# nelpy/ghost

Hardware: NVIDIA B200
Metric: cwt_output_coeffs_per_sec (higher is better)
Workload: dtype f32

## Files before the change

### ghost_b200/csrc/fast_path.cu

```cuda
#include "plan.h"
#include "common.cuh"
#include "multiplier.cuh"
#include <algorithm>
#include <atomic>
#include <cmath>
#include <cstdio>
#include <cstdlib>
#include <map>
#include <type_traits>

namespace gcwt {

constexpr int kMaxFastLevel = 14;
constexpr int kMaxFullScales = 64;
constexpr double kMaxHaloFrac = 0.45;

__constant__ float c_halfband[kHalfbandOdd];
constexpr int kSmallCoef = (2 + 4 + 8) * kInterpT;
__constant__ float c_interp_small[kSmallCoef];
constexpr int kWideCoef = (4 + 8) * kWideT;
__constant__ float c_interp_wide[kWideCoef];

static double bessel_i0(double x) {
    double sum = 1.0, term = 1.0;
    const double q = x * x / 4.0;
    for (int k = 1; k < 200; ++k) {
        term *= q / ((double)k * (double)k);
        sum += term;
        if (term < 1e-18 * sum) break;
    }
    return sum;
}

static void design_halfband(double* odd ) {
    const int T = kHalfbandT;
    const double atten = 140.0;
    const double beta = 0.1102 * (atten - 8.7);
    const double i0b = bessel_i0(beta);
    double sum = 0.0;
    for (int k = 0; k < kHalfbandOdd; ++k) {
        const int t = 2 * k + 1;
        const double r = (double)t / (double)T;
        const double win = bessel_i0(beta * std::sqrt(std::max(0.0, 1.0 - r * r))) / i0b;
        const double x = M_PI * t / 2.0;
        odd[k] = 0.5 * std::sin(x) / x * win;
        sum += 2.0 * odd[k];
    }
    for (int k = 0; k < kHalfbandOdd; ++k) odd[k] *= 0.5 / sum;
    long double done = 0.0L;
    for (int k = 0; k < kHalfbandOdd; ++k) {
        long double rest = 0.0L;
        for (int j = k + 1; j < kHalfbandOdd; ++j) rest += (long double)odd[j];
        const float f = (float)(0.25L - done - rest);
        odd[k] = (double)f;
        done += (long double)f;
    }
}

static double halfband_gain(const double* odd, double theta) {
    double g = 0.5;
    for (int k = 0; k < kHalfbandOdd; ++k) g += 2.0 * (double)(float)odd[k] * std::cos((2 * k + 1) * theta);
    return g;
}

constexpr int kPlanLevels = kMaxFastLevel - kMinFastLevel + 1;
constexpr int kWide2Levels = kWideMaxLevel - kMinFastLevel + 1;
constexpr int kPlanRow = kPlanLevels * kBins + kFullN + kWide2Levels * 2 * kBins;
// ... 11 lines not shown
        const int k = i - kPlanLevels * kBins - kFullN;
        n = (int64_t)(2 * kChunkDec) << (kMinFastLevel + k / (2 * kBins)); m = k % (2 * kBins);
    }
    out[(int64_t)s * kPlanRow + i] = morse_response(m, n, sc.L, sc.k_first, sc.n_terms, terms + sc.term_off);
}

struct PlanResponses {
    std::vector<double> g;
    const double* level(int s, int lev) const { return g.data() + (size_t)s * kPlanRow + (size_t)(lev - kMinFastLevel) * kBins; }
    const double* full(int s) const { return g.data() + (size_t)s * kPlanRow + (size_t)kPlanLevels * kBins; }
    const double* wide2(int s, int lev) const {
        return g.data() + (size_t)s * kPlanRow + (size_t)kPlanLevels * kBins + kFullN + (size_t)(lev - kMinFastLevel) * 2 * kBins;
    }
};

static int compute_plan_responses(const gcwt_plan* p, PlanResponses& pr) {
    const size_t count = (size_t)p->n_scales * kPlanRow;
    double* d = nullptr;
    GCWT_CUDA_OK(cudaMalloc((void**)&d, sizeof(double) * count));
    plan_response_kernel<<<dim3((kPlanRow + 127) / 128, p->n_scales), 128>>>(p->d_scales, p->d_terms, d);
    count_launch();
    pr.g.resize(count);
    cudaError_t e = cudaMemcpy(pr.g.data(), d, sizeof(double) * count, cudaMemcpyDeviceToHost);
    cudaFree(d);
    if (e != cudaSuccess) { set_error(std::string("plan responses: ") + cudaGetErrorString(e)); return GCWT_ERR_CUDA; }
    return GCWT_OK;
}

static double filter_energy(const gcwt_plan* p, const ScaleInfo& sc, int64_t n) {
    const double* X = p->terms.data() + sc.term_off;
    double e = 0.0;
    for (int t = 0; t < sc.n_terms; ++t) e += X[t] * X[t];
    return e * (double)n / (double)sc.L;
}

static bool band_fits(const gcwt_plan* p, const PlanResponses& pr, int s, int level) {
    const double* g = pr.level(s, level);
    double e_in = 0.0;
    for (int m = 0; m < kBins; ++m) e_in += g[m] * g[m];
    const double e_tot = filter_energy(p, p->scales[s], (int64_t)kChunkDec << level);
    return (1.0 - e_in / e_tot) < p->band_tol * p->band_tol;
}

static int full_extent(const gcwt_plan* p, const PlanResponses& pr, int s) {
    const double* g = pr.full(s);
    const double e_tot = filter_energy(p, p->scales[s], kFullN);
    double e_in = 0.0;
    int m = 0;
    for (int nmu = 2; nmu <= 8; nmu *= 2) {
        for (; m < nmu * kBins; ++m) e_in += g[m] * g[m];
        if ((1.0 - e_in / e_tot) < p->band_tol * p->band_tol) return nmu;
    }
    return 16;
}

static int band_width_bins(const gcwt_plan* p, const PlanResponses& pr, int s, int level) {
    const double* g = pr.level(s, level);
    const double e_tot = filter_energy(p, p->scales[s], (int64_t)kChunkDec << level);
    const double budget = 0.5 * p->band_tol * p->band_tol * e_tot;
    int lo = 0, hi = kBins - 1;
    double acc = 0.0;
    while (lo < hi && acc + g[lo] * g[lo] < budget) { acc += g[lo] * g[lo]; ++lo; }
    acc = 0.0;
    while (hi > lo && acc + g[hi] * g[hi] < budget) { acc += g[hi] * g[hi]; --hi; }
    return hi - lo + 1;
}

static int choose_level(const gcwt_plan* p, const PlanResponses& pr, int s) {
    const ScaleInfo& sc = p->scales[s];
    if (!(p->flags & GCWT_FLAG_FORCE_GENERIC)) {
        int lo = kMinFastLevel;
        while (lo <= kMaxFastLevel && (double)(sc.L - 1) > kMaxHaloFrac * (double)((int64_t)kChunkDec << lo)) ++lo;
        int hi = std::min(kMaxFastLevel, ilog2_ceil(sc.L) + 1);
        for (int lev = hi; lev >= lo; --lev)
            if (band_fits(p, pr, s, lev)) return lev;
        if ((double)(sc.L - 1) <= kMaxHaloFrac * kFullN) return -1;
    }
    return -2;
}

static void class_geometry(FastClass& fc) {
    const int64_t d = fc.level >= 0 ? (int64_t(1) << fc.level) : 1;
    const int64_t align = std::max<int64_t>(d, 16);
    const int taps = fc.wide ? kWideT : kInterpT;
    const int64_t lead = fc.interp ? (int64_t)(taps / 2 - 1) << fc.log2u : 0;
    const int64_t tail = fc.interp ? (int64_t)(taps / 2 + 1) << fc.log2u : 0;
    fc.offset = ((fc.lmax / 2 + lead + align - 1) / align) * align;
    fc.hop = ((fc.nc_full - (fc.lmax - 1) / 2 - tail - fc.offset) / align) * align;
}

static long double sinc_pi(long double x) {
    const long double pi = 3.14159265358979323846264338327950288L;
    return x == 0.0L ? 1.0L : sinl(pi * x) / (pi * x);
}

static void design_interpolator(int log2u, std::vector<float>& coef, int T, double os) {
    const int U = 1 << log2u;
    const long double fmax = 0.5L / (long double)os;
    coef.resize((size_t)U * T);
    std::vector<long double> A((size_t)T * T), b(T);
    for (int t = 0; t < T; ++t) coef[t] = (t == T / 2 - 1) ? 1.f : 0.f;
    for (int phi = 1; phi < U; ++phi) {
        for (int t = 0; t < T; ++t) {
            const long double dt = (long double)(t - (T / 2 - 1)) - (long double)phi / U;
            for (int u = 0; u < T; ++u) A[(size_t)t * T + u] = sinc_pi(2.0L * fmax * (long double)(t - u));
            b[t] = sinc_pi(2.0L * fmax * dt);
// ... 106 lines not shown
            const double step = 2.0 * pi / (double)sc.L;
            double far = 0.0, near = 0.0;
            for (int q = 0; q < sc.n_terms; ++q) {
                const int64_t k = sc.k_first + q;
                const double d = w - step * (double)k;
                if (fabs(d) < step) near += X[q];
                else far += ((k & 1) ? -X[q] : X[q]) / sin(0.5 * d);
            }
            const double v = 1.15 * (fabs(far) / (double)sc.L + near);
            atomicMax(&mx[b], __float_as_uint((float)v));
        }
    }
    __syncthreads();
    if (tid < kGuardSlots) out[(int64_t)s * kGuardSlots + tid] = __uint_as_float(mx[tid]);
}

static int guard_plan_build(gcwt_plan* p, const PlanResponses& pr, const std::vector<double>& hb) {
    const int S = p->n_scales;
    std::vector<float> gain((size_t)S * kGuardSlots, 0.f), q(S, 0.f);
    std::vector<int32_t> cls(S, -1);
    for (size_t ci = 0; ci < p->classes.size(); ++ci)
        for (int id : p->classes[ci].scale_ids) cls[id] = (int32_t)ci;
    GCWT_CUDA_OK(cudaMemcpy(p->d_scales, p->scales.data(), sizeof(ScaleInfo) * S, cudaMemcpyHostToDevice));
    float* d_drop = nullptr;
    GCWT_CUDA_OK(cudaMalloc((void**)&d_drop, sizeof(float) * S * kGuardSlots));
    guard_drop_kernel<<<S, 256>>>(p->d_scales, p->d_terms, d_drop);
    count_launch();
    std::vector<float> drop((size_t)S * kGuardSlots);
    cudaError_t e = cudaMemcpy(drop.data(), d_drop, sizeof(float) * drop.size(), cudaMemcpyDeviceToHost);
    cudaFree(d_drop);
    if (e != cudaSuccess) { set_error(std::string("guard tables: ") + cudaGetErrorString(e)); return GCWT_ERR_CUDA; }
    HbTaps taps;
    for (int k = 0; k < kHalfbandOdd; ++k) taps.odd[k] = (double)(float)p->halfband_odd[k];
    std::map<int, std::vector<float>> alias;
    for (const FastClass& fc : p->classes) {
        if (fc.level < kMinFastLevel || alias.count(fc.level)) continue;
        unsigned* d_b = nullptr;
        GCWT_CUDA_OK(cudaMalloc((void**)&d_b, sizeof(unsigned) * kGuardSlots * kBins));
        GCWT_CUDA_OK(cudaMemset(d_b, 0, sizeof(unsigned) * kGuardSlots * kBins));
        const int64_t total = (int64_t)kBins << fc.level;
        guard_alias_kernel<<<(unsigned)((total + 255) / 256), 256>>>(fc.level, taps, d_b);
        count_launch();
        std::vector<float>& B = alias[fc.level];
        B.resize((size_t)kGuardSlots * kBins);
        e = cudaMemcpy(B.data(), d_b, sizeof(float) * B.size(), cudaMemcpyDeviceToHost);
        cudaFree(d_b);
        if (e != cudaSuccess) { set_error(std::string("guard tables: ") + cudaGetErrorString(e)); return GCWT_ERR_CUDA; }
    }
    for (int s = 0; s < S; ++s) {
        const int lev = p->scales[s].level;
        if (cls[s] < 0) continue;
        if (lev < 0) {
            const double* g = pr.full(s);
            double acc = 0.0;
            for (int m = 0; m < kFullN; ++m) acc += g[m] * g[m];
            q[s] = (float)(acc / kFullN);
            continue;
        }
        const double* g = pr.level(s, lev);
        const std::vector<float>& B = alias[lev];
        double T[kBins], acc = 0.0;
        for (int m = 0; m < kBins; ++m) {
            double t = std::fabs(g[m]);
            for (int j = 1; j <= lev; ++j) t /= hb[(size_t)j * kBins + m];
            T[m] = t;
            acc += t * t;
        }
        q[s] = (float)(acc / kChunkDec);
        for (int b = 0; b <= lev + 1 && b < kGuardSlots; ++b) {
            double al = 0.0;
            if (b < lev)
                for (int m = 0; m < kBins; ++m) al = std::max(al, (double)B[(size_t)b * kBins + m] * T[m]);
            const double tot = al + (double)drop[(size_t)s * kGuardSlots + b];
            gain[(size_t)s * kGuardSlots + b] = (float)(tot * tot);
        }
    }
    GCWT_CUDA_OK(cudaMalloc((void**)&p->d_guard_gain, sizeof(float) * gain.size()));
    GCWT_CUDA_OK(cudaMalloc((void**)&p->d_guard_q, sizeof(float) * S));
    GCWT_CUDA_OK(cudaMalloc((void**)&p->d_guard_class, sizeof(int32_t) * S));
    GCWT_CUDA_OK(cudaMemcpy(p->d_guard_gain, gain.data(), sizeof(float) * gain.size(), cudaMemcpyHostToDevice));
    GCWT_CUDA_OK(cudaMemcpy(p->d_guard_q, q.data(), sizeof(float) * S, cudaMemcpyHostToDevice));
    GCWT_CUDA_OK(cudaMemcpy(p->d_guard_class, cls.data(), sizeof(int32_t) * S, cudaMemcpyHostToDevice));
    GCWT_CUDA_OK(cudaEventCreateWithFlags(&p->ev_guard, cudaEventDisableTiming));
    p->guard_last_flags.assign(S, 0);
    p->guard_gain_h = gain;
    p->guard_q_h = q;
    return GCWT_OK;
}

int fast_plan_build(gcwt_plan* p) {
    design_halfband(p->halfband_odd);
    { int rc = upload_constants(p); if (rc) return rc; }
    {
        std::vector<float2> tw(kFullN);
        for (int k = 0; k < kFullN; ++k) {
            const double a = -2.0 * M_PI * (double)k / (double)kFullN;
            tw[k] = make_float2((float)std::cos(a), (float)std::sin(a));
        }
        GCWT_CUDA_OK(cudaMalloc((void**)&p->d_twiddle, sizeof(float2) * kFullN));
        GCWT_CUDA_OK(cudaMemcpy(p->d_twiddle, tw.data(), sizeof(float2) * kFullN, cudaMemcpyHostToDevice));
    }
    PlanResponses pr;
    { int rc = compute_plan_responses(p, pr); if (rc) return rc; }
    std::vector<double> hb((size_t)(kMaxFastLevel + 1) * kBins, 1.0);
    for (int j = 1; j <= kMaxFastLevel; ++j)
        for (int m = 0; m < kBins; ++m)
            hb[(size_t)j * kBins + m] = halfband_gain(p->halfband_odd, 2.0 * M_PI * (double)m / (double)((int64_t)kChunkDec << j));
    std::map<int, std::vector<int>> by_level;
    p->max_level = 0;
    for (int s = 0; s < p->n_scales; ++s) {
        ScaleInfo& sc = p->scales[s];
        sc.level = choose_level(p, pr, s);
        if (sc.level == -2) p->generic_ids.push_back(s);
        else by_level[sc.level].push_back(s);
        p->max_level = std::max(p->max_level, sc.level);
    }
    for (auto& kv : by_level) {
        const int level = kv.first;
        const std::vector<int>& ids = kv.second;
        const int cap = level >= 0 ? kMaxClassScales : kMaxFullScales;
        for (size_t i0 = 0; i0 < ids.size(); i0 += cap) {
            p->classes.emplace_back();
            FastClass& fc = p->classes.back();
            fc.level = level;
            fc.nc_full = level >= 0 ? ((int64_t)kChunkDec << level) : kFullN;
            fc.scale_ids.assign(ids.begin() + i0, ids.begin() + std::min(ids.size(), i0 + cap));
            fc.lmax = 1;
            for (int id : fc.scale_ids) fc.lmax = std::max(fc.lmax, p->scales[id].L);
            const bool may_interp = p->out_kind != GCWT_OUT_COMPLEX && !(p->flags & GCWT_FLAG_NO_INTERP);
            fc.interp = level >= kInterpMinLevel && may_interp;
            fc.log2u = level - 1;
            int wmax = 1;
            if (level >= 0)
                for (int id : fc.scale_ids) wmax = std::max(wmax, band_width_bins(p, pr, id, level));
            if (may_interp && level >= 2 && level <= kWideMaxLevel) {
                if (512.0 / (double)wmax >= kWideMinOs) { fc.interp = true; fc.wide = true; fc.log2u = level; }
            }
            class_geometry(fc);
            if (fc.hop <= 0) { set_error("planner: non-positive hop"); return GCWT_ERR_ARG; }
            if (fc.wide) {
                const int64_t d = int64_t(1) << level, align = std::max<int64_t>(d, 16), nc2 = 2 * fc.nc_full;
                const int64_t lead = (int64_t)(kWideT / 2 - 1) << fc.log2u, tail = (int64_t)(kWideT / 2 + 1) << fc.log2u;
                fc.offset2 = ((fc.lmax / 2 + lead + align - 1) / align) * align;
                fc.hop2 = ((nc2 - (fc.lmax - 1) / 2 - tail - fc.offset2) / align) * align;
                const int ns2 = (int)fc.scale_ids.size();
                std::vector<float2> tab2((size_t)ns2 * 2 * kBins);
                for (int i = 0; i < ns2; ++i) {
                    const ScaleInfo& sc = p->scales[fc.scale_ids[i]];
                    const double* gsrc = pr.wide2(fc.scale_ids[i], level);
                    for (int m = 0; m < 2 * kBins; ++m) {
                        double g = gsrc[m] / (double)(2 * kChunkDec);
                        for (int j = 1; j <= level; ++j)
                            g /= halfband_gain(p->halfband_odd, 2.0 * M_PI * (double)m / (double)((int64_t)(2 * kChunkDec) << j));
                        double re = g, im = 0.0;
                        if ((sc.L & 1) == 0) {
                            const double ph = -M_PI * (double)m / (double)nc2;
                            re = g * std::cos(ph);
                            im = g * std::sin(ph);
                        }
                        tab2[(size_t)i * 2 * kBins + m] = make_float2((float)re, (float)im);
                    }
                }
                GCWT_CUDA_OK(cudaMalloc((void**)&fc.d_table2, sizeof(float2) * tab2.size()));
                GCWT_CUDA_OK(cudaMemcpy(fc.d_table2, tab2.data(), sizeof(float2) * tab2.size(), cudaMemcpyHostToDevice));
            }
            const int nb = level >= 0 ? kBins : kFullN;
            const int ns = (int)fc.scale_ids.size();
            std::vector<float2> tab((size_t)ns * nb);
            for (int i = 0; i < ns; ++i) {
                const ScaleInfo& sc = p->scales[fc.scale_ids[i]];
                const double* gsrc = level >= 0 ? pr.level(fc.scale_ids[i], level) : pr.full(fc.scale_ids[i]);
                for (int m = 0; m < nb; ++m) {
                    double g = gsrc[m];
                    if (level >= 0) {
                        for (int j = 1; j <= level; ++j) g /= hb[(size_t)j * kBins + m];
                        g /= (double)kChunkDec;
                    } else {
                        g /= (double)kFullN;
                    }
                    double re = g, im = 0.0;
                    if ((sc.L & 1) == 0) {
                        const double ph = -M_PI * (double)m / (double)fc.nc_full;
                        re = g * std::cos(ph);
                        im = g * std::sin(ph);
                    }
                    tab[(size_t)i * nb + m] = make_float2((float)re, (float)im);
                }
            }
            GCWT_CUDA_OK(cudaMalloc((void**)&fc.d_table, sizeof(float2) * tab.size()));
            GCWT_CUDA_OK(cudaMemcpy(fc.d_table, tab.data(), sizeof(float2) * tab.size(), cudaMemcpyHostToDevice));
            if (fc.interp) {
                std::vector<float> coef;
                if (fc.wide) {
                    design_interpolator(fc.log2u, coef, kWideT, kWideMinOs);
                } else {
                    const double os = std::min(8.0, std::max(kInterpMinOs, 0.98 * 1024.0 / (double)wmax));
                    design_interpolator(fc.log2u, coef, kInterpT, os);
                }
                GCWT_CUDA_OK(cudaMalloc((void**)&fc.d_coef, sizeof(float) * coef.size()));
                GCWT_CUDA_OK(cudaMemcpy(fc.d_coef, coef.data(), sizeof(float) * coef.size(), cudaMemcpyHostToDevice));
            }
            if (level < 0) {
                for (int id : fc.scale_ids) fc.scale_nmu.push_back(full_extent(p, pr, id));
                GCWT_CUDA_OK(cudaMalloc((void**)&fc.d_scale_nmu, sizeof(int32_t) * ns));
                GCWT_CUDA_OK(cudaMemcpy(fc.d_scale_nmu, fc.scale_nmu.data(), sizeof(int32_t) * ns, cudaMemcpyHostToDevice));
            }
            GCWT_CUDA_OK(cudaMalloc((void**)&fc.d_scale_ids, sizeof(int32_t) * ns));
            GCWT_CUDA_OK(cudaMemcpy(fc.d_scale_ids, fc.scale_ids.data(), sizeof(int32_t) * ns, cudaMemcpyHostToDevice));
        }
    }
    if (p->guard && !p->classes.empty()) {
        if (p->max_level + 2 >= kGuardLevels || (int)p->classes.size() > 64) p->guard = false;
        else { int rc = guard_plan_build(p, pr, hb); if (rc) return rc; }
    } else {
        p->guard = false;
    }
    return GCWT_OK;
}

void fast_plan_free(gcwt_plan* p) {
    if (p->d_guard_gain) cudaFree(p->d_guard_gain);
    if (p->d_guard_q) cudaFree(p->d_guard_q);
    if (p->d_guard_class) cudaFree(p->d_guard_class);
    if (p->d_guard_acc) cudaFree(p->d_guard_acc);
    if (p->d_guard_pow) cudaFree(p->d_guard_pow);
    if (p->d_guard_flags) cudaFree(p->d_guard_flags);
    if (p->h_guard_flags) cudaFreeHost(p->h_guard_flags);
    if (p->ev_guard) cudaEventDestroy(p->ev_guard);
    p->d_guard_gain = p->d_guard_q = nullptr; p->d_guard_class = nullptr; p->d_guard_acc = nullptr;
    p->d_guard_pow = nullptr; p->d_guard_flags = p->h_guard_flags = nullptr; p->ev_guard = nullptr;
    for (auto& fc : p->classes) {
        if (fc.d_table) cudaFree(fc.d_table);
        if (fc.d_table2) cudaFree(fc.d_table2);
        if (fc.d_scale_ids) cudaFree(fc.d_scale_ids);
        if (fc.d_coef) cudaFree(fc.d_coef);
        if (fc.d_scale_nmu) cudaFree(fc.d_scale_nmu);
    }
    p->classes.clear();
}

constexpr int kPyrTile = 1024;

template <typename TIn, bool FIRST>
__global__ void __launch_bounds__(256)
pyramid_kernel(const TIn* __restrict__ in, int64_t in_stride, int64_t in_lo, int64_t in_hi,
               const double* __restrict__ means, float* __restrict__ out, int64_t out_stride,
               int64_t out_lo, int64_t out_len,
               double* __restrict__ acc, int acc_stride, int level, int64_t seg_in, int64_t seg_out) {
    static_assert(kHalfbandT == 19, "tile indexing below assumes kMid == 9");
    constexpr int kMid = (kHalfbandT - 1) / 2;
    constexpr int kEv = kPyrTile + 2 * kMid + 2 + 4;
    constexpr int kOdShift = 12 - kMid;
    __shared__ __align__(16) float ev[kEv];
    __shared__ __align__(16) float ods[kEv + 16];
    const int c = blockIdx.y;
    const int64_t i0 = out_lo + (int64_t)blockIdx.x * kPyrTile;
// ... 45 lines not shown
        }
        *(float4*)(out + (int64_t)c * out_stride + (i0 + j0 - out_lo)) = make_float4(o[0], o[1], o[2], o[3]);
    }
    if (acc != nullptr) {
#pragma unroll
        for (int o = 16; o > 0; o >>= 1) {
            e_out += __shfl_xor_sync(0xffffffffu, e_out, o);
            if (FIRST) e_in += __shfl_xor_sync(0xffffffffu, e_in, o);
        }
        __syncthreads();
        if ((threadIdx.x & 31) == 0) { ev[threadIdx.x >> 5] = e_out; if (FIRST) ev[8 + (threadIdx.x >> 5)] = e_in; }
        __syncthreads();
        if (threadIdx.x == 0) {
            double* a = acc + (int64_t)c * acc_stride;
            float so = 0.f, si = 0.f;
#pragma unroll
            for (int w = 0; w < 8; ++w) { so += ev[w]; if (FIRST) si += ev[8 + w]; }
            if (so != 0.f) atomicAdd(a + level, (double)so);
            if (FIRST && si != 0.f) atomicAdd(a, (double)si);
        }
    }
}

struct FusedParams {
    const void* src;
    int64_t src_stride;
    int64_t src_lo, src_hi;
    const double* means;
    int log2d;
    int p_cols;
    int log2p;
    float inv_nc;
    int64_t offset, hop, n_chunks, n;
    int n_scales;
    const int32_t* scale_ids;
    const float2* table;
    void* out;
    int64_t s_stride, c_stride;
    int iters;
    int units_per_chunk;
    int log2u;
    const float* coef;
    const float2* twf;
    const int32_t* scale_nmu;
    double* acc;
    int acc_stride;
    int class_idx;
    float ech_weight;
    float* pow;
    int pow_stride;
    float pow_weight;
    int guard_every;
    int q_mode;
};

__device__ __forceinline__ float2 tw_pos(const float2* __restrict__ twf, int k) {
    const float2 t = __ldg(twf + (k & (kFullN - 1)));
    return make_float2(t.x, -t.y);
}

__device__ __forceinline__ float sqrt_abs_approx(float v) {
    float r;
    asm("sqrt.approx.ftz.f32 %0, %1;" : "=f"(r) : "f"(fabsf(v)));
    return r;
}

__device__ __forceinline__ float sqrt_approx(float v) {
    float r;
    asm("sqrt.approx.ftz.f32 %0, %1;" : "=f"(r) : "f"(v));
    return r;
}

template <int KIND> struct out_elem { typedef float type; };
template <> struct out_elem<GCWT_OUT_COMPLEX> { typedef float2 type; };

__device__ __forceinline__ void st_pred(float* p, float v, unsigned on) {
#ifdef GCWT_EXP_CSSTORE
    asm volatile("{\n\t.reg .pred q;\n\tsetp.ne.b32 q, %2, 0;\n\t@q st.global.cs.f32 [%0], %1;\n\t}"
                 :: "l"(p), "f"(v), "r"(on) : "memory");
    return;
#endif
    asm volatile("{\n\t.reg .pred q;\n\tsetp.ne.b32 q, %2, 0;\n\t@q st.global.f32 [%0], %1;\n\t}"
                 :: "l"(p), "f"(v), "r"(on) : "memory");
}
__device__ __forceinline__ void st_pred(float2* p, float2 v, unsigned on) {
    asm volatile("{\n\t.reg .pred q;\n\tsetp.ne.b32 q, %3, 0;\n\t@q st.global.v2.f32 [%0], {%1, %2};\n\t}"
                 :: "l"(p), "f"(v.x), "f"(v.y), "r"(on) : "memory");
}

template <int KIND>
__device__ __forceinline__ void store_column(typename out_elem<KIND>::type* __restrict__ op, int64_t stride,
                                             unsigned mask, const float2* a) {
#pragma unroll
    for (int k = 0; k < 16; ++k) {
        const unsigned on = mask & (1u << k);
        if constexpr (KIND == GCWT_OUT_COMPLEX) st_pred(op + k * stride, a[k], on);
        else if constexpr (KIND == GCWT_OUT_AMPLITUDE) st_pred(op + k * stride, sqrt_approx(a[k].x * a[k].x + a[k].y * a[k].y), on);
        else st_pred(op + k * stride, a[k].x * a[k].x + a[k].y * a[k].y, on);
    }
}

__device__ __forceinline__ unsigned valid_mask(int rel, int sh, int lo, int hi) {
    const int step = 1 << sh;
    int k_lo = (lo - rel + step - 1) >> sh;
    int k_hi = (hi - rel + step - 1) >> sh;
    k_lo = max(k_lo, 0);
// ... 824 lines not shown
    int* s_ids = (int*)(A + kTileA);
    int* s_nmu = s_ids + kMaxFullScales;
    float* s_pow = (float*)(s_nmu + kMaxFullScales);

    const int tid = threadIdx.x;
    if (tid < 2) s_pow[tid] = 0.f;
    const int r = tid & 15;
    const int g = tid >> 4;
    const int64_t qi = blockIdx.x % prm.n_chunks;
    const int64_t c = blockIdx.x / prm.n_chunks;
    const int64_t q = prm.q_mode == 0 ? qi : (prm.q_mode == 1 ? qi * prm.guard_every : qi + qi / (prm.guard_every - 1) + 1);
    const int64_t t0 = q * prm.hop - prm.offset;

    {
        const TIn* src = (const TIn*)prm.src + c * prm.src_stride;
        const double mu = prm.means[c];
        TIn raw[kFullN / 256];
        unsigned inside = 0;
#pragma unroll
        for (int k = 0; k < kFullN / 256; ++k) {
            const int64_t u = t0 + tid + 256 * k;
            const bool ok = u >= prm.src_lo && u < prm.src_hi;
            raw[k] = ok ? src[u] : (TIn)0;
            inside |= (unsigned)ok << k;
        }
        float val[kFullN / 256];
#pragma unroll
        for (int k = 0; k < kFullN / 256; ++k)
            val[k] = (inside >> k & 1) ? (float)((double)raw[k] - mu) : 0.f;
        const float cm = chunk_mean<kFullN / 256>(val, (float*)ex + 2048);
        if (GUARD)
            chunk_energy_add<kFullN / 256>(val, cm, (float*)ex + 2048, prm.acc + c * prm.acc_stride + kGuardLevels + prm.class_idx,
                                           prm.ech_weight);
#pragma unroll
        for (int k = 0; k < kFullN / 256; ++k) A[tid + 256 * k] = make_float2(val[k] - cm, 0.f);
        __syncthreads();
        smem_fft4096_forward(A, Yf, prm.twf);
    }
    float2 tw[16], tw4k[16];
#pragma unroll
    for (int k = 0; k < 16; ++k) {
        tw[k] = tw_pos(prm.twf, 16 * g * k);
        tw4k[k] = tw_pos(prm.twf, tid * k);
    }
    typedef typename out_elem<KIND>::type OutT;
    const int rel = g * 16 + r;
    const unsigned mask = valid_mask(rel, 8, (int)prm.offset, (int)min(prm.offset + prm.hop, prm.n - t0));
    OutT* const out_c = (OutT*)prm.out + c * prm.c_stride + t0;
    if (tid < prm.n_scales) { s_ids[tid] = prm.scale_ids[tid]; s_nmu[tid] = prm.scale_nmu[tid]; }
    __syncthreads();
    full_scale_loop<KIND, GUARD>(prm, Yf, ex, A, s_ids, s_nmu, s_pow, tw, tw4k, out_c, rel, mask);
}

template <int KIND, int LP, bool GUARD>
static void launch_banded_g(unsigned nblk, cudaStream_t st, const FusedParams& prm) {
    static std::atomic<bool> attr_set[64];
    int dev = 0;
    cudaGetDevice(&dev);
    if (!attr_set[dev & 63]) {
        cudaFuncSetAttribute(fused_banded_kernel<KIND, LP, GUARD>, cudaFuncAttributeMaxDynamicSharedMemorySize, (int)kBandedSmem);
        attr_set[dev & 63] = true;
    }
    fused_banded_kernel<KIND, LP, GUARD><<<nblk, 256, kBandedSmem, st>>>(prm);
}

template <int KIND, int LP>
static void launch_banded_one(unsigned nblk, cudaStream_t st, const FusedParams& prm) {
    if (prm.pow != nullptr) launch_banded_g<KIND, LP, true>(nblk, st, prm);
    else launch_banded_g<KIND, LP, false>(nblk, st, prm);
}

static void launch_banded(int kind, int lp, unsigned nblk, cudaStream_t st, const FusedParams& prm) {
    if (kind == GCWT_OUT_COMPLEX) {
        if (lp == 4) launch_banded_one<GCWT_OUT_COMPLEX, 4>(nblk, st, prm);
        else launch_banded_one<GCWT_OUT_COMPLEX, 0>(nblk, st, prm);
    } else if (kind == GCWT_OUT_AMPLITUDE) {
        if (lp == 4) launch_banded_one<GCWT_OUT_AMPLITUDE, 4>(nblk, st, prm);
        else launch_banded_one<GCWT_OUT_AMPLITUDE, 0>(nblk, st, prm);
    } else {
        if (lp == 4) launch_banded_one<GCWT_OUT_POWER, 4>(nblk, st, prm);
        else launch_banded_one<GCWT_OUT_POWER, 0>(nblk, st, prm);
    }
}

template <typename TIn, int KIND, bool GUARD>
static void launch_full_g(unsigned nblk, cudaStream_t st, const FusedParams& prm) {
    static std::atomic<bool> attr_set[64];
    int dev = 0;
    cudaGetDevice(&dev);
    if (!attr_set[dev & 63]) {
        cudaFuncSetAttribute(fused_full_kernel<TIn, KIND, GUARD>, cudaFuncAttributeMaxDynamicSharedMemorySize, (int)kFullSmem);
        attr_set[dev & 63] = true;
    }
    fused_full_kernel<TIn, KIND, GUARD><<<nblk, 256, kFullSmem, st>>>(prm);
}

template <typename TIn, int KIND>
static void launch_full_kind(unsigned nblk, cudaStream_t st, const FusedParams& prm, bool measure) {
    if (measure) launch_full_g<TIn, KIND, true>(nblk, st, prm);
    else launch_full_g<TIn, KIND, false>(nblk, st, prm);
}

template <typename TIn>
static void launch_full(int kind, unsigned nblk, cudaStream_t st, const FusedParams& prm, bool measure) {
    if (kind == GCWT_OUT_COMPLEX) launch_full_kind<TIn, GCWT_OUT_COMPLEX>(nblk, st, prm, measure);
    else if (kind == GCWT_OUT_AMPLITUDE) launch_full_kind<TIn, GCWT_OUT_AMPLITUDE>(nblk, st, prm, measure);
    else launch_full_kind<TIn, GCWT_OUT_POWER>(nblk, st, prm, measure);
}

struct LevelGeom { int64_t lo, hi, len, stride; float* ptr; };

template <typename TIn>
static int fast_run(gcwt_plan* p, const TIn* x, int in_type, int64_t n_channels, int64_t n,
                    int64_t x_stride, int64_t halo_l, int64_t halo_r, const double* d_means,
                    void* out, int64_t s_stride, int64_t c_stride, cudaStream_t st) {
    const bool guard = p->guard;
    const int acc_stride = kGuardLevels + (int)p->classes.size();
    if (guard) {
        if (p->guard_cap < n_channels) {
            if (p->d_guard_acc) cudaFree(p->d_guard_acc);
            if (p->d_guard_pow) cudaFree(p->d_guard_pow);
            if (p->d_guard_flags) cudaFree(p->d_guard_flags);
            if (p->h_guard_flags) cudaFreeHost(p->h_guard_flags);
            p->d_guard_acc = nullptr; p->d_guard_pow = nullptr; p->d_guard_flags = p->h_guard_flags = nullptr; p->guard_cap = 0;
            GCWT_CUDA_OK(cudaMalloc((void**)&p->d_guard_acc, sizeof(double) * acc_stride * n_channels));
            GCWT_CUDA_OK(cudaMalloc((void**)&p->d_guard_pow, sizeof(float) * p->n_scales * n_channels));
            GCWT_CUDA_OK(cudaMalloc((void**)&p->d_guard_flags, (size_t)p->n_scales * n_channels));
            GCWT_CUDA_OK(cudaMallocHost((void**)&p->h_guard_flags, (size_t)p->n_scales * n_channels));
            p->guard_cap = n_channels;
        }
        GCWT_CUDA_OK(cudaMemsetAsync(p->d_guard_acc, 0, sizeof(double) * acc_stride * n_channels, st));
        GCWT_CUDA_OK(cudaMemsetAsync(p->d_guard_pow, 0, sizeof(float) * p->n_scales * n_channels, st));
    }
    const int levels = std::max(p->max_level, 0) + ((guard && p->max_level > 0) ? 2 : 0);
    std::vector<LevelGeom> lv(levels + 1);
    lv[0].lo = -halo_l; lv[0].hi = n + halo_r;
    size_t total = 0;
    for (int j = 1; j <= levels; ++j) {
        const int64_t plo = lv[j - 1].lo, phi = lv[j - 1].hi - 1;
        const int64_t lo = (int64_t)std::floor((double)(plo - kHalfbandT) / 2.0);
        const int64_t hi = (int64_t)std::ceil((double)(phi + kHalfbandT) / 2.0);
        lv[j].lo = lo; lv[j].hi = hi + 1; lv[j].len = hi - lo + 1;
        lv[j].stride = (lv[j].len + 3) & ~int64_t(3);
        total += (size_t)lv[j].stride * n_channels;
    }
    int rc = ensure_workspace(p, total * sizeof(float) + 256);
    if (rc) return rc;
    float* w = (float*)p->ws.ptr;
    for (int j = 1; j <= levels; ++j) { lv[j].ptr = w; w += lv[j].stride * n_channels; }

    const int sp_pyr = prof_begin(p, 0, st);
    for (int j = 1; j <= levels; ++j) {
        dim3 grid((unsigned)((lv[j].len + kPyrTile - 1) / kPyrTile), (unsigned)n_channels);
        double* acc = guard ? p->d_guard_acc : nullptr;
        const int64_t seg_in = (n + (int64_t(1) << (j - 1)) - 1) >> (j - 1), seg_out = (n + (int64_t(1) << j) - 1) >> j;
        if (j == 1)
            pyramid_kernel<TIn, true><<<grid, 256, 0, st>>>(x, x_stride, lv[0].lo, lv[0].hi, d_means, lv[1].ptr,
                                                            lv[1].stride, lv[1].lo, lv[1].len, acc, acc_stride, j,
                                                            seg_in, seg_out);
        else
// ... 44 lines not shown
            prm.offset = fc.offset2; prm.hop = fc.hop2;
            prm.n_chunks = (n + fc.hop2 - 1) / fc.hop2;
            prm.table = fc.d_table2;
            set_guard_sampling(prm.n_chunks, 8, (double)(int64_t(1) << fc.level) * (double)fc.hop2 / (double)(2 * fc.nc_full));
            prm.p_cols = 8; prm.log2p = 3; prm.units_per_chunk = 1;
            prm.iters = rows_aligned32 ? 2 : (rows_aligned ? 1 : 0);
            const int64_t nblk = n_channels * prm.n_chunks;
            if (nblk > 0x7fffffffLL) { set_error("fast path: grid too large"); return GCWT_ERR_UNSUPPORTED; }
            if (p->out_kind == GCWT_OUT_AMPLITUDE) {
                if (guard) fused_wide2_kernel<GCWT_OUT_AMPLITUDE, true><<<(unsigned)nblk, 256, kWide2Smem, cs>>>(prm);
                else fused_wide2_kernel<GCWT_OUT_AMPLITUDE, false><<<(unsigned)nblk, 256, kWide2Smem, cs>>>(prm);
            } else {
                if (guard) fused_wide2_kernel<GCWT_OUT_POWER, true><<<(unsigned)nblk, 256, kWide2Smem, cs>>>(prm);
                else fused_wide2_kernel<GCWT_OUT_POWER, false><<<(unsigned)nblk, 256, kWide2Smem, cs>>>(prm);
            }
        } else if (uses_interp(fc)) {
            const LevelGeom& g = lv[fc.level];
            prm.src = g.ptr; prm.src_stride = g.stride; prm.src_lo = g.lo; prm.src_hi = g.hi;
            prm.log2d = fc.level;
            prm.p_cols = (int)(fc.nc_full / kBins);
            prm.log2p = ilog2_ceil(prm.p_cols);
            prm.iters = rows_aligned32 ? 2 : 1;
            const int64_t chunks = n_channels * prm.n_chunks;
            int64_t splits = (1776 + chunks - 1) / chunks;
            splits = std::max<int64_t>(1, std::min<int64_t>(splits, std::max<int64_t>(1, (int64_t(1) << fc.level) / 32)));
            splits = std::min<int64_t>(splits, 24);
            prm.units_per_chunk = (int)splits;
            const int64_t nblk = chunks * splits;
            if (nblk > 0x7fffffffLL) { set_error("fast path: grid too large"); return GCWT_ERR_UNSUPPORTED; }
            if (p->out_kind == GCWT_OUT_AMPLITUDE) {
                if (guard) fused_interp_kernel<GCWT_OUT_AMPLITUDE, true><<<(unsigned)nblk, 256, kInterpSmem, cs>>>(prm);
                else fused_interp_kernel<GCWT_OUT_AMPLITUDE, false><<<(unsigned)nblk, 256, kInterpSmem, cs>>>(prm);
            } else {
                if (guard) fused_interp_kernel<GCWT_OUT_POWER, true><<<(unsigned)nblk, 256, kInterpSmem, cs>>>(prm);
                else fused_interp_kernel<GCWT_OUT_POWER, false><<<(unsigned)nblk, 256, kInterpSmem, cs>>>(prm);
            }
        } else if (fc.level >= 0) {
            const LevelGeom& g = lv[fc.level];
            prm.src = g.ptr; prm.src_stride = g.stride; prm.src_lo = g.lo; prm.src_hi = g.hi;
            prm.log2d = fc.level;
            prm.p_cols = (int)(fc.nc_full / kBins);
            prm.log2p = ilog2_ceil(prm.p_cols);
            const int blocks = prm.p_cols / 16;
            prm.iters = std::min(blocks, 16);
            prm.units_per_chunk = (blocks + prm.iters - 1) / prm.iters;
            const int64_t nblk = n_channels * prm.n_chunks * prm.units_per_chunk;
            if (nblk > 0x7fffffffLL) { set_error("fast path: grid too large"); return GCWT_ERR_UNSUPPORTED; }
            launch_banded(p->out_kind, prm.log2p, (unsigned)nblk, cs, prm);
        } else {
            prm.src = x; prm.src_stride = x_stride; prm.src_lo = -halo_l; prm.src_hi = n + halo_r;
            prm.log2d = 0; prm.p_cols = 16; prm.log2p = 4; prm.iters = 1; prm.units_per_chunk = 1;
            const int64_t nblk = n_channels * prm.n_chunks;
            if (nblk > 0x7fffffffLL) { set_error("fast path: grid too large"); return GCWT_ERR_UNSUPPORTED; }
            if (!guard) {
                launch_full<TIn>(p->out_kind, (unsigned)nblk, cs, prm, false);
            } else {
                const int64_t n_all = prm.n_chunks, n_meas = (n_all + prm.guard_every - 1) / prm.guard_every;
                if (n_all > n_meas) {
                    prm.q_mode = 2; prm.n_chunks = n_all - n_meas;
                    launch_full<TIn>(p->out_kind, (unsigned)(n_channels * prm.n_chunks), cs, prm, false);
                    count_launch();
                }
                prm.q_mode = prm.guard_every > 1 ? 1 : 0; prm.n_chunks = n_meas;
                launch_full<TIn>(p->out_kind, (unsigned)(n_channels * prm.n_chunks), full_meas_stream ? full_meas_stream : cs, prm, true);
            }
        }
        count_launch();
        prof_end(p, sp, cs);
        return GCWT_OK;
    };

    bool side0_pending = false;
    if (guard && !p->profile && getenv("GCWT_STREAMS") == nullptr) {
        if (!p->side_stream[0]) {
            GCWT_CUDA_OK(cudaStreamCreateWithFlags(&p->side_stream[0], cudaStreamNonBlocking));
            GCWT_CUDA_OK(cudaEventCreateWithFlags(&p->ev_join[0], cudaEventDisableTiming));
        }
        if (!p->ev_fork) GCWT_CUDA_OK(cudaEventCreateWithFlags(&p->ev_fork, cudaEventDisableTiming));
        GCWT_CUDA_OK(cudaEventRecord(p->ev_fork, st));
        GCWT_CUDA_OK(cudaStreamWaitEvent(p->side_stream[0], p->ev_fork, 0));
        full_meas_stream = p->side_stream[0];
        side0_pending = true;
    }
    int n_group = 0;
    for (const FastClass& fc : p->classes) {
        if (uses_interp(fc)) { ++n_group; continue; }
        rc = launch_class(fc, st, true);
        if (rc) return rc;
    }
    if (n_group > 0) {
        int n_streams = 2;
        if (const char* e = getenv("GCWT_STREAMS")) n_streams = std::max(1, std::min(1 + gcwt_plan::kSideStreams, atoi(e)));
        const bool per_class = p->profile && getenv("GCWT_CLASS_TIMES") != nullptr;
        if (per_class || n_group < 2) n_streams = 1;
        const int n_side = n_streams - 1;
        for (int k = 0; k < n_side; ++k) {
            if (!p->side_stream[k]) {
                GCWT_CUDA_OK(cudaStreamCreateWithFlags(&p->side_stream[k], cudaStreamNonBlocking));
                GCWT_CUDA_OK(cudaEventCreateWithFlags(&p->ev_join[k], cudaEventDisableTiming));
            }
        }
        if (n_side > 0 && !p->ev_fork) GCWT_CUDA_OK(cudaEventCreateWithFlags(&p->ev_fork, cudaEventDisableTiming));
        const int sp = per_class ? -1 : prof_begin(p, 4, st, 63);
        if (n_side > 0) {
            GCWT_CUDA_OK(cudaEventRecord(p->ev_fork, st));
            for (int k = 0; k < n_side; ++k) GCWT_CUDA_OK(cudaStreamWaitEvent(p->side_stream[k], p->ev_fork, 0));
        }
        int ci = 0;
        for (const FastClass& fc : p->classes) {
            if (!uses_interp(fc)) continue;
            const int slot = ci++ % n_streams;
            rc = launch_class(fc, slot ? p->side_stream[slot - 1] : st, per_class);
            if (rc) return rc;
        }
        for (int k = 0; k < n_side; ++k) {
            GCWT_CUDA_OK(cudaEventRecord(p->ev_join[k], p->side_stream[k]));
            GCWT_CUDA_OK(cudaStreamWaitEvent(st, p->ev_join[k], 0));
// ... 149 lines not shown
```

### ghost_b200/csrc/plan.h

```cpp
#pragma once
#include <cuda_runtime.h>
#include <stdint.h>
#include <vector>
#include "../../include/ghost_cwt.h"

namespace gcwt {

constexpr int kBins = 256;
constexpr int kChunkDec = 1024;
constexpr int kFullN = 4096;
#ifndef GCWT_MAX_CLASS
#define GCWT_MAX_CLASS 16
#endif
#ifndef GCWT_INTERP_T
#define GCWT_INTERP_T 8
#endif
#ifndef GCWT_WIDE_T
#define GCWT_WIDE_T 12
#endif
#ifndef GCWT_INTERP_CTAS
#define GCWT_INTERP_CTAS 2
#endif
constexpr int kMaxClassScales = GCWT_MAX_CLASS;
constexpr int kMinFastLevel = 2;
constexpr int kInterpT = GCWT_INTERP_T;
constexpr int kInterpMinLevel = 3;
constexpr int kCoarse = 2048;
constexpr int kWideT = GCWT_WIDE_T;
constexpr int kWideMaxLevel = 3;
constexpr double kInterpMinOs = 4.0;
constexpr double kWideMinOs = 2.5;
constexpr int kHalfbandT = 19;
constexpr int kHalfbandOdd = (kHalfbandT + 1) / 2;

struct ScaleInfo {
    int64_t L;
    int32_t k_first;
    int32_t n_terms;
    int32_t term_off;
    int32_t level;
};

struct FastClass {
    int level = 0;
    int64_t nc_full = 0;
    int64_t lmax = 0;
    int64_t offset = 0;
    int64_t hop = 0;
    std::vector<int> scale_ids;
    float2* d_table = nullptr;
    int32_t* d_scale_ids = nullptr;
    std::vector<int> scale_nmu;
    int32_t* d_scale_nmu = nullptr;
    bool interp = false;
    bool wide = false;
    float2* d_table2 = nullptr;
    int64_t offset2 = 0, hop2 = 0;
    int log2u = 0;
    float* d_coef = nullptr;
};

constexpr int kGuardSlots = 18;
constexpr int kGuardLevels = 20;
constexpr double kGuardKRound = 6.0;
constexpr double kGuardKStage = 2.0;

struct Workspace {
    void* ptr = nullptr;
    size_t bytes = 0;
};

}

struct gcwt_plan {
    int n_scales = 0;
    int compute_type = GCWT_F32;
    int out_kind = GCWT_OUT_AMPLITUDE;
    int device = 0;
    int flags = 0;
    double band_tol = 1e-7;
    std::vector<gcwt::ScaleInfo> scales;
    std::vector<double> terms;
    gcwt::ScaleInfo* d_scales = nullptr;
    double* d_terms = nullptr;
    std::vector<gcwt::FastClass> classes;
    std::vector<int> generic_ids;
    int max_level = 0;
    double halfband_odd[gcwt::kHalfbandOdd];
    gcwt::Workspace ws;
    bool profile = false;
    struct Span { cudaEvent_t a, b; int kind; int launches; int tag; };
    std::vector<Span> spans;
    double prof_ms[GCWT_PROFILE_KINDS] = {0, 0, 0, 0, 0};
    double class_ms[64] = {0};
    int64_t prof_launches[GCWT_PROFILE_KINDS] = {0, 0, 0, 0, 0};
    float2* d_twiddle = nullptr;
    double* d_means = nullptr;
// ... 70 lines not shown
```

Before: 771.0 billion.

## Add 1024-point full-band FFT class for short-support scales

Scales on the full-band (level -1) path whose support L fits the halo limit are now grouped into a new class that uses a 1024-point transform instead of the 4096-point one. A new fused kernel handles two chunks per block: it runs a shared-memory 1024-point forward FFT, a pruned 32x32 inverse FFT per scale, and twiddled transposes through padded warp tiles. The aim is to cut FFT work and shared memory per output for short wavelets. The cost is a smaller hop per chunk, which means more halo overhead and more chunks. The filter tables and extents are built by subsampling the 4096-point responses.

```diff
diff --git a/ghost_b200/csrc/fast_path.cu b/ghost_b200/csrc/fast_path.cu
--- a/ghost_b200/csrc/fast_path.cu
+++ b/ghost_b200/csrc/fast_path.cu
@@ -13,6 +13,7 @@
 
 constexpr int kMaxFastLevel = 14;
 constexpr int kMaxFullScales = 64;
+constexpr int kFull1kN = 1024;
 constexpr double kMaxHaloFrac = 0.45;
 
 __constant__ float c_halfband[kHalfbandOdd];
@@ -130,6 +131,25 @@
         if ((1.0 - e_in / e_tot) < p->band_tol * p->band_tol) return nmu;
     }
     return 16;
+}
+
+static int full1k_extent(const gcwt_plan* p, const PlanResponses& pr, int s) {
+    const double* g = pr.full(s);
+    const double e_tot = filter_energy(p, p->scales[s], kFull1kN);
+    double e_in = 0.0;
+    int m = 0;
+    for (int nmu = 2; nmu <= 16; nmu *= 2) {
+        for (; m < nmu * 32; ++m) e_in += g[4 * m] * g[4 * m];
+        if ((1.0 - e_in / e_tot) < p->band_tol * p->band_tol) return nmu;
+    }
+    return 32;
+}
+
+constexpr int64_t kFull1kMaxL = 1024;
+static int64_t full1k_max_l() {
+    int64_t v = kFull1kMaxL;
+    if (const char* e = getenv("GCWT_FULL1K_MAXL")) v = atoll(e);
+    return std::min<int64_t>(v, (int64_t)(kMaxHaloFrac * kFull1kN) + 1);
 }
 
 static int band_width_bins(const gcwt_plan* p, const PlanResponses& pr, int s, int level) {
@@ -342,9 +362,10 @@
         if (cls[s] < 0) continue;
         if (lev < 0) {
             const double* g = pr.full(s);
+            const int step = p->classes[cls[s]].full1k ? kFullN / kFull1kN : 1;
             double acc = 0.0;
-            for (int m = 0; m < kFullN; ++m) acc += g[m] * g[m];
-            q[s] = (float)(acc / kFullN);
+            for (int m = 0; m < kFullN; m += step) acc += g[m] * g[m];
+            q[s] = (float)(acc * step / kFullN);
             continue;
         }
         const double* g = pr.level(s, lev);
@@ -398,6 +419,7 @@
             hb[(size_t)j * kBins + m] = halfband_gain(p->halfband_odd, 2.0 * M_PI * (double)m / (double)((int64_t)kChunkDec << j));
     std::map<int, std::vector<int>> by_level;
     p->max_level = 0;
+    const int64_t max_l_1k = full1k_max_l();
     for (int s = 0; s < p->n_scales; ++s) {
         ScaleInfo& sc = p->scales[s];
         sc.level = choose_level(p, pr, s);
@@ -405,15 +427,24 @@
         else by_level[sc.level].push_back(s);
         p->max_level = std::max(p->max_level, sc.level);
     }
+    struct Group { int level; bool full1k; std::vector<int> ids; };
+    std::vector<Group> groups;
     for (auto& kv : by_level) {
-        const int level = kv.first;
-        const std::vector<int>& ids = kv.second;
+        if (kv.first >= 0) { groups.push_back({kv.first, false, kv.second}); continue; }
+        Group g1k{-1, true, {}}, g4k{-1, false, {}};
+        for (int id : kv.second) (p->scales[id].L <= max_l_1k ? g1k : g4k).ids.push_back(id);
+        for (Group* g : {&g1k, &g4k}) if (!g->ids.empty()) groups.push_back(*g);
+    }
+    for (const Group& grp : groups) {
+        const int level = grp.level;
+        const std::vector<int>& ids = grp.ids;
         const int cap = level >= 0 ? kMaxClassScales : kMaxFullScales;
         for (size_t i0 = 0; i0 < ids.size(); i0 += cap) {
             p->classes.emplace_back();
             FastClass& fc = p->classes.back();
             fc.level = level;
-            fc.nc_full = level >= 0 ? ((int64_t)kChunkDec << level) : kFullN;
+            fc.full1k = grp.full1k;
+            fc.nc_full = level >= 0 ? ((int64_t)kChunkDec << level) : (fc.full1k ? kFull1kN : kFullN);
             fc.scale_ids.assign(ids.begin() + i0, ids.begin() + std::min(ids.size(), i0 + cap));
             fc.lmax = 1;
             for (int id : fc.scale_ids) fc.lmax = std::max(fc.lmax, p->scales[id].L);
@@ -454,19 +485,20 @@
                 GCWT_CUDA_OK(cudaMalloc((void**)&fc.d_table2, sizeof(float2) * tab2.size()));
                 GCWT_CUDA_OK(cudaMemcpy(fc.d_table2, tab2.data(), sizeof(float2) * tab2.size(), cudaMemcpyHostToDevice));
             }
-            const int nb = level >= 0 ? kBins : kFullN;
+            const int nb = level >= 0 ? kBins : (int)fc.nc_full;
+            const int stride = level >= 0 ? 1 : kFullN / nb;
             const int ns = (int)fc.scale_ids.size();
             std::vector<float2> tab((size_t)ns * nb);
             for (int i = 0; i < ns; ++i) {
                 const ScaleInfo& sc = p->scales[fc.scale_ids[i]];
                 const double* gsrc = level >= 0 ? pr.level(fc.scale_ids[i], level) : pr.full(fc.scale_ids[i]);
                 for (int m = 0; m < nb; ++m) {
-                    double g = gsrc[m];
+                    double g = gsrc[stride * m];
                     if (level >= 0) {
                         for (int j = 1; j <= level; ++j) g /= hb[(size_t)j * kBins + m];
                         g /= (double)kChunkDec;
                     } else {
-                        g /= (double)kFullN;
+                        g /= (double)nb;
                     }
                     double re = g, im = 0.0;
                     if ((sc.L & 1) == 0) {
@@ -491,7 +523,7 @@
                 GCWT_CUDA_OK(cudaMemcpy(fc.d_coef, coef.data(), sizeof(float) * coef.size(), cudaMemcpyHostToDevice));
             }
             if (level < 0) {
-                for (int id : fc.scale_ids) fc.scale_nmu.push_back(full_extent(p, pr, id));
+                for (int id : fc.scale_ids) fc.scale_nmu.push_back(fc.full1k ? full1k_extent(p, pr, id) : full_extent(p, pr, id));
                 GCWT_CUDA_OK(cudaMalloc((void**)&fc.d_scale_nmu, sizeof(int32_t) * ns));
                 GCWT_CUDA_OK(cudaMemcpy(fc.d_scale_nmu, fc.scale_nmu.data(), sizeof(int32_t) * ns, cudaMemcpyHostToDevice));
             }
@@ -643,6 +675,7 @@
     float pow_weight;
     int guard_every;
     int q_mode;
+    int64_t n_units;
 };
 
 __device__ __forceinline__ float2 tw_pos(const float2* __restrict__ twf, int k) {
@@ -1573,6 +1606,198 @@
     full_scale_loop<KIND, GUARD>(prm, Yf, ex, A, s_ids, s_nmu, s_pow, tw, tw4k, out_c, rel, mask);
 }
 
+constexpr int kFull1kChunks = 2;
+constexpr int kTile1k = 32 * 33;
+constexpr size_t kFull1kSmem = sizeof(float2) * (kFull1kChunks * kFull1kN + 8 * kTile1k) + sizeof(int64_t) * 2 * kFull1kChunks;
+
+template <int SIGN>
+__device__ __forceinline__ float2 mul_w32(float2 a, int e) {
+    e &= 31;
+    if (e == 0) return a;
+    if (e == 16) return make_float2(-a.x, -a.y);
+    if (e == 8) return mul_i<SIGN>(a);
+    if (e == 24) return mul_i<-SIGN>(a);
+    const float c[9] = {1.f, 0.98078528040323044913f, 0.92387953251128675613f, 0.83146961230254523708f,
+                        0.70710678118654752440f, 0.55557023301960222474f, 0.38268343236508977173f,
+                        0.19509032201612826785f, 0.f};
+    const int q = e >> 3, r = e & 7;
+    float x, y;
+    if (q == 0) { x = c[r]; y = c[8 - r]; }
+    else if (q == 1) { x = -c[8 - r]; y = c[r]; }
+    else if (q == 2) { x = -c[r]; y = -c[8 - r]; }
+    else { x = c[8 - r]; y = -c[r]; }
+    return cmul(a, make_float2(x, SIGN > 0 ? y : -y));
+}
+
+template <int SIGN>
+__device__ __forceinline__ void dft32(float2* a) {
+    float2 e[16], o[16];
+#pragma unroll
+    for (int k = 0; k < 16; ++k) { e[k] = a[2 * k]; o[k] = a[2 * k + 1]; }
+    dft16<SIGN>(e);
+    dft16<SIGN>(o);
+#pragma unroll
+    for (int k = 0; k < 16; ++k) {
+        const float2 t = mul_w32<SIGN>(o[k], k);
+        a[k] = cadd(e[k], t);
+        a[k + 16] = csub(e[k], t);
+    }
+}
+
+template <int NMU>
+__device__ __forceinline__ void pruned_idft32(const float2* in, float2* out) {
+    if constexpr (NMU == 32) {
+#pragma unroll
+        for (int k = 0; k < 32; ++k) out[k] = in[k];
+        dft32<+1>(out);
+    } else {
+        constexpr int R = 32 / NMU;
+#pragma unroll
+        for (int kb = 0; kb < R; ++kb) {
+            float2 v[NMU];
+#pragma unroll
+            for (int mu = 0; mu < NMU; ++mu) v[mu] = mul_w32<+1>(in[mu], mu * kb);
+            small_dft<NMU, +1, float2>::run(v);
+#pragma unroll
+            for (int ka = 0; ka < NMU; ++ka) out[ka * R + kb] = v[ka];
+        }
+    }
+}
+
+template <int NMU>
+__device__ __forceinline__ void full1k_stage1(const float2* __restrict__ Y, const float2* __restrict__ tab, float2* b) {
+    float2 z[NMU];
+#pragma unroll
+    for (int mu = 0; mu < NMU; ++mu) z[mu] = cmul(Y[32 * mu], __ldg(tab + 32 * mu));
+    pruned_idft32<NMU>(z, b);
+}
+
+__device__ __forceinline__ unsigned valid_mask32(int rel, int lo, int hi) {
+    int j_lo = (lo - rel + 31) >> 5;
+    int j_hi = (hi - rel + 31) >> 5;
+    j_lo = max(j_lo, 0);
+    j_hi = min(max(j_hi, 0), 32);
+    if (j_hi <= j_lo) return 0u;
+    const unsigned below_hi = j_hi == 32 ? 0xffffffffu : ((1u << j_hi) - 1u);
+    return below_hi & ~((1u << j_lo) - 1u);
+}
+
+template <typename TIn, int KIND, bool GUARD>
+__global__ void __launch_bounds__(256, 2)
+fused_full1k_kernel(const FusedParams prm) {
+    extern __shared__ __align__(16) unsigned char smem_raw[];
+    float2* Y = (float2*)smem_raw;
+    float2* tiles = Y + kFull1kChunks * kFull1kN;
+    int64_t* s_c = (int64_t*)(tiles + 8 * kTile1k);
+    int64_t* s_t0 = s_c + kFull1kChunks;
+    const int tid = threadIdx.x;
+    const int lane = tid & 31, warp = tid >> 5;
+
+    int64_t cc[kFull1kChunks], t0s[kFull1kChunks];
+    int n_valid = 0;
+#pragma unroll
+    for (int h = 0; h < kFull1kChunks; ++h) {
+        const int64_t lin = (int64_t)blockIdx.x * kFull1kChunks + h;
+        const int64_t qi = lin % prm.n_chunks;
+        const int64_t q = prm.q_mode == 0 ? qi : (prm.q_mode == 1 ? qi * prm.guard_every : qi + qi / (prm.guard_every - 1) + 1);
+        cc[h] = lin / prm.n_chunks;
+        t0s[h] = q * prm.hop - prm.offset;
+        n_valid += lin < prm.n_units;
+    }
+    if (tid == 0) {
+#pragma unroll
+        for (int h = 0; h < kFull1kChunks; ++h) { s_c[h] = cc[h]; s_t0[h] = t0s[h]; }
+    }
+    {
+        TIn raw[kFull1kChunks][kFull1kN / 256];
+        unsigned inside = 0;
+#pragma unroll
+        for (int h = 0; h < kFull1kChunks; ++h) {
+            const TIn* src = (const TIn*)prm.src + (h < n_valid ? cc[h] : 0) * prm.src_stride;
+#pragma unroll
+            for (int k = 0; k < kFull1kN / 256; ++k) {
+                const int64_t u = t0s[h] + tid + 256 * k;
+                const bool ok = h < n_valid && u >= prm.src_lo && u < prm.src_hi;
+                raw[h][k] = ok ? src[u] : (TIn)0;
+                inside |= (unsigned)ok << (h * 4 + k);
+            }
+        }
+        float* scratch = (float*)(tiles + kFull1kN);
+#pragma unroll
+        for (int h = 0; h < kFull1kChunks; ++h) {
+            if (h >= n_valid) break;
+            const double mu = prm.means[cc[h]];
+            float val[kFull1kN / 256];
+#pragma unroll
+            for (int k = 0; k < kFull1kN / 256; ++k)
+                val[k] = (inside >> (h * 4 + k) & 1) ? (float)((double)raw[h][k] - mu) : 0.f;
+            const float cm = chunk_mean<kFull1kN / 256>(val, scratch);
+            if (GUARD)
+                chunk_energy_add<kFull1kN / 256>(val, cm, scratch, prm.acc + cc[h] * prm.acc_stride + kGuardLevels + prm.class_idx,
+                                                 prm.ech_weight);
+#pragma unroll
+            for (int k = 0; k < kFull1kN / 256; ++k) tiles[tid + 256 * k] = make_float2(val[k] - cm, 0.f);
+            __syncthreads();
+            smem_fft1024_forward(tiles, Y + h * kFull1kN, prm.twf);
+        }
+    }
+    float2 wb[8];
+#pragma unroll
+    for (int b = 1; b < 8; ++b) wb[b] = tw_pos(prm.twf, 4 * lane * b);
+
+    typedef typename out_elem<KIND>::type OutT;
+    float2* tile = tiles + warp * kTile1k;
+    const int n_items = n_valid * prm.n_scales;
+    for (int item = warp; item < n_items; item += 8) {
+        const int s = n_valid == 2 ? item >> 1 : item;
+        const int h = item - s * n_valid;
+        const int nmu = __ldg(prm.scale_nmu + s);
+        const float2* Yh = Y + h * kFull1kN + lane;
+        const float2* tab = prm.table + (int64_t)s * kFull1kN + lane;
+        float2 b[32];
+        if (nmu == 2) full1k_stage1<2>(Yh, tab, b);
+        else if (nmu == 4) full1k_stage1<4>(Yh, tab, b);
+        else if (nmu == 8) full1k_stage1<8>(Yh, tab, b);
+        else if (nmu == 16) full1k_stage1<16>(Yh, tab, b);
+        else full1k_stage1<32>(Yh, tab, b);
+        float2 wa[4];
+        wa[1] = cmul(wb[4], wb[4]);
+        wa[2] = cmul(wa[1], wa[1]);
+        wa[3] = cmul(wa[2], wa[1]);
+        __syncwarp();
+#pragma unroll
+        for (int k = 0; k < 32; ++k) {
+            const int a = k >> 3, bb = k & 7;
+            const float2 w = bb == 0 ? wa[a] : (a == 0 ? wb[bb] : cmul(wa[a], wb[bb]));
+            tile[lane * 33 + k] = k == 0 ? b[k] : cmul(b[k], w);
+        }
+        __syncwarp();
+#pragma unroll
+        for (int m = 0; m < 32; ++m) b[m] = tile[m * 33 + lane];
+        dft32<+1>(b);
+        const int64_t c = s_c[h];
+        const int64_t t0 = s_t0[h];
+        const unsigned mask = valid_mask32(lane, (int)prm.offset, (int)min(prm.offset + prm.hop, prm.n - t0));
+        const int sid = __ldg(prm.scale_ids + s);
+        OutT* op = (OutT*)prm.out + c * prm.c_stride + (int64_t)sid * prm.s_stride + t0 + lane;
+#pragma unroll
+        for (int j = 0; j < 32; ++j) {
+            const unsigned on = mask & (1u << j);
+            if constexpr (KIND == GCWT_OUT_COMPLEX) st_pred(op + 32 * j, b[j], on);
+            else if constexpr (KIND == GCWT_OUT_AMPLITUDE) st_pred(op + 32 * j, sqrt_approx(b[j].x * b[j].x + b[j].y * b[j].y), on);
+            else st_pred(op + 32 * j, b[j].x * b[j].x + b[j].y * b[j].y, on);
+        }
+        if (GUARD) {
+            float pw = 0.f;
+#pragma unroll
+            for (int j = 0; j < 32; ++j) pw += (mask >> j & 1u) ? b[j].x * b[j].x + b[j].y * b[j].y : 0.f;
+#pragma unroll
+            for (int o = 16; o > 0; o >>= 1) pw += __shfl_xor_sync(0xffffffffu, pw, o);
+            if (lane == 0) atomicAdd(prm.pow + c * prm.pow_stride + sid, pw * prm.pow_weight);
+        }
+    }
+}
+
 template <int KIND, int LP, bool GUARD>
 static void launch_banded_g(unsigned nblk, cudaStream_t st, const FusedParams& prm) {
     static std::atomic<bool> attr_set[64];
@@ -1627,6 +1852,33 @@
     if (kind == GCWT_OUT_COMPLEX) launch_full_kind<TIn, GCWT_OUT_COMPLEX>(nblk, st, prm, measure);
     else if (kind == GCWT_OUT_AMPLITUDE) launch_full_kind<TIn, GCWT_OUT_AMPLITUDE>(nblk, st, prm, measure);
     else launch_full_kind<TIn, GCWT_OUT_POWER>(nblk, st, prm, measure);
+}
+
+template <typename TIn, int KIND, bool GUARD>
+static void launch_full1k_g(unsigned nblk, cudaStream_t st, const FusedParams& prm) {
+    static std::atomic<bool> attr_set[64];
+    int dev = 0;
+    cudaGetDevice(&dev);
+    if (!attr_set[dev & 63]) {
+        cudaFuncSetAttribute(fused_full1k_kernel<TIn, KIND, GUARD>, cudaFuncAttributeMaxDynamicSharedMemorySize, (int)kFull1kSmem);
+        attr_set[dev & 63] = true;
+    }
+    fused_full1k_kernel<TIn, KIND, GUARD><<<nblk, 256, kFull1kSmem, st>>>(prm);
+}
+
+template <typename TIn>
+static void launch_full1k(int kind, cudaStream_t st, const FusedParams& prm, bool measure) {
+    const unsigned nblk = (unsigned)((prm.n_units + kFull1kChunks - 1) / kFull1kChunks);
+    if (kind == GCWT_OUT_COMPLEX) {
+        if (measure) launch_full1k_g<TIn, GCWT_OUT_COMPLEX, true>(nblk, st, prm);
+        else launch_full1k_g<TIn, GCWT_OUT_COMPLEX, false>(nblk, st, prm);
+    } else if (kind == GCWT_OUT_AMPLITUDE) {
+        if (measure) launch_full1k_g<TIn, GCWT_OUT_AMPLITUDE, true>(nblk, st, prm);
+        else launch_full1k_g<TIn, GCWT_OUT_AMPLITUDE, false>(nblk, st, prm);
+    } else {
+        if (measure) launch_full1k_g<TIn, GCWT_OUT_POWER, true>(nblk, st, prm);
+        else launch_full1k_g<TIn, GCWT_OUT_POWER, false>(nblk, st, prm);
+    }
 }
 
 struct LevelGeom { int64_t lo, hi, len, stride; float* ptr; };
@@ -1777,17 +2029,22 @@
             prm.log2d = 0; prm.p_cols = 16; prm.log2p = 4; prm.iters = 1; prm.units_per_chunk = 1;
             const int64_t nblk = n_channels * prm.n_chunks;
             if (nblk > 0x7fffffffLL) { set_error("fast path: grid too large"); return GCWT_ERR_UNSUPPORTED; }
+            auto launch = [&](cudaStream_t ls, bool measure) {
+                prm.n_units = n_channels * prm.n_chunks;
+                if (fc.full1k) launch_full1k<TIn>(p->out_kind, ls, prm, measure);
+                else launch_full<TIn>(p->out_kind, (unsigned)prm.n_units, ls, prm, measure);
+            };
             if (!guard) {
-                launch_full<TIn>(p->out_kind, (unsigned)nblk, cs, prm, false);
+                launch(cs, false);
             } else {
                 const int64_t n_all = prm.n_chunks, n_meas = (n_all + prm.guard_every - 1) / prm.guard_every;
                 if (n_all > n_meas) {
                     prm.q_mode = 2; prm.n_chunks = n_all - n_meas;
-                    launch_full<TIn>(p->out_kind, (unsigned)(n_channels * prm.n_chunks), cs, prm, false);
+                    launch(cs, false);
                     count_launch();
                 }
                 prm.q_mode = prm.guard_every > 1 ? 1 : 0; prm.n_chunks = n_meas;
-                launch_full<TIn>(p->out_kind, (unsigned)(n_channels * prm.n_chunks), full_meas_stream ? full_meas_stream : cs, prm, true);
+                launch(full_meas_stream ? full_meas_stream : cs, true);
             }
         }
         count_launch();
diff --git a/ghost_b200/csrc/plan.h b/ghost_b200/csrc/plan.h
--- a/ghost_b200/csrc/plan.h
+++ b/ghost_b200/csrc/plan.h
@@ -43,6 +43,7 @@
 
 struct FastClass {
     int level = 0;
+    bool full1k = false;
     int64_t nc_full = 0;
     int64_t lmax = 0;
     int64_t offset = 0;
```

Result: slower. 729.8 billion, median of 6 (-5.3%).
